# PhilippBongartz/RepeatResolver

Hardware: AMD Instinct MI355X
Metric: sum-of-pairs DP cells/sec (higher is better)
Workload: dtype u32

## Files before the change

repeatresolver_amd/csrc/pwr_device.hip:

```cpp
#include <hip/hip_runtime.h>

#include <algorithm>
#include <chrono>
#include <cstdint>
#include <cstdio>
#include <cstdlib>
#include <cstring>
#include <new>
#include <thread>
#include <type_traits>
#include <vector>

#include "pwr.h"

#define PWR_INF 0x40000000u
#define PWR_BIG 0x7fffffff

struct Hdr {
    int W;
    int nslots;
    int nfree;
    int cur;
    int status;
    int stop;
// ... 62 lines not shown
    Tally *tally;
    int *order0, *order1;
    int *rank;
    int *freelist;
    const long long *brkoff;
    const int *brkx;
    int *nbrk;
    int *hard;
    int *inscnt;
    int *newidx;
    int *bplan;
};
#define PLAN_MAX 16
#define JR_BASE (1 + 2 * PLAN_MAX)
#define BPLAN_WORDS (JR_BASE + 64 * 4)
#define PLAN_CAND 128
#define PLAN_EVRATE_MAX 12.0f
#define PLAN_SLACK 2048

#define SEG_MAX 256
struct SegDesc {
    int job, s;
    int xb, xown, xe;
    int fin, active;
    int grow0;
    unsigned long long cells;
};
struct GatherPart;
struct CommitJob {
    int nchg, nev, ndel, first;
    int u0, u1;
    int scanned, pad;
};
struct BatchPlan;
struct CommitEv;
struct JobBufs {
    GatherPart *gpart;
    unsigned gather_tag;
    JobMeta *meta;
    int *way;
    int4 *rec2;
    uint8_t *mark;
    uint8_t *mark2;
    uint32_t *dirs;
    int *newcol;
    int *aux;
    uint4 *desc;
    int wpNW, wpMS;
    unsigned *lastM;
    unsigned long long *gmb;
    SegDesc *seg;
    unsigned *chk;
    int seg_align;
    int src_start;
    int smax, seg_rows, warm_cols;
    int seg_budget, seg_minrows;
    int seg_balance;
    int plan_ahead;
    int hard_rows, hard_up, hard_down;
    int plan_len;
    int plan_gate_rel;
    int spec_inorder;
    int fail_stops;
    int plan_slack, plan_evrate_x100;
    const int *rowids;
    int gstride;
    unsigned tagbase;
    unsigned long long *gtr;
    int trk;
    unsigned trace_tag;
    long long *g64;
    int force64;
    int evcap;
    int gate_v2;
    int *chkdone;
    int check_in_trace, trace_ny;
    int trace_prior;
    int trace_blk;
    int v2_follows, f64_follows;
    int stall_test;
    unsigned long long *diag;
    int njobs_launched;
    int Lmax, colcap, NC;
    size_t dirstride;
    int split_rank, split_world;
    CommitJob *cjob;
    int *chg;
    int *evkey, *evdl;
    int *insidx;
    int *pair_cf, *pair_left;
    BatchPlan *plan;
    CommitEv *sev;
    int *freed;
    unsigned *ticket;
};
#define NOT_MINE(JB, JOB) ((JB).split_world > 1 && (JOB) % (JB).split_world != (JB).split_rank)

#define DPP_ROW_SHR(n) (0x110 + (n))
#define DPP_ROW_BCAST15 0x142
#define DPP_ROW_BCAST31 0x143
#define DPP_WAVE_SHR1 0x138

__device__ __forceinline__ int wave_incl_min(int v)
{
    int t;
    t = __builtin_amdgcn_update_dpp(PWR_BIG, v, DPP_ROW_SHR(1), 0xF, 0xF, false); v = min(v, t);
    t = __builtin_amdgcn_update_dpp(PWR_BIG, v, DPP_ROW_SHR(2), 0xF, 0xF, false); v = min(v, t);
    t = __builtin_amdgcn_update_dpp(PWR_BIG, v, DPP_ROW_SHR(4), 0xF, 0xF, false); v = min(v, t);
    t = __builtin_amdgcn_update_dpp(PWR_BIG, v, DPP_ROW_SHR(8), 0xF, 0xF, false); v = min(v, t);
    t = __builtin_amdgcn_update_dpp(PWR_BIG, v, DPP_ROW_BCAST15, 0xA, 0xF, false); v = min(v, t);
    t = __builtin_amdgcn_update_dpp(PWR_BIG, v, DPP_ROW_BCAST31, 0xC, 0xF, false); v = min(v, t);
    return v;
}
__device__ __forceinline__ int row_incl_min(int v)
{
    int t;
    t = __builtin_amdgcn_update_dpp(PWR_BIG, v, DPP_ROW_SHR(1), 0xF, 0xF, false); v = min(v, t);
    t = __builtin_amdgcn_update_dpp(PWR_BIG, v, DPP_ROW_SHR(2), 0xF, 0xF, false); v = min(v, t);
    t = __builtin_amdgcn_update_dpp(PWR_BIG, v, DPP_ROW_SHR(4), 0xF, 0xF, false); v = min(v, t);
    t = __builtin_amdgcn_update_dpp(PWR_BIG, v, DPP_ROW_SHR(8), 0xF, 0xF, false); v = min(v, t);
    return v;
}
__device__ __forceinline__ unsigned wave_incl_add(unsigned v)
{
    unsigned t;
    t = __builtin_amdgcn_update_dpp(0u, v, DPP_ROW_SHR(1), 0xF, 0xF, false); v += t;
// ... 2524 lines not shown
        for (int j = lane; j < nch; j += 64)
            tot += (int)((__hip_atomic_load(&hand[j], __ATOMIC_RELAXED, __HIP_MEMORY_SCOPE_AGENT) >> 41) & 0x7full);
        for (int o = 32; o > 0; o >>= 1) tot += __shfl_xor(tot, o);
        if (lane == 0) m->nnew = tot;
    }
#undef TB_POST
}

#define COMMIT_NT 1024
#define EVCAP 1024
#define MAXJ 128
#define CS_G 16
#define CA_G 32

__device__ __forceinline__ int row_symbol(const uint8_t *mk, int y, int lo, int y0, int y1)
{
    if (y < y0 || y > y1) return 5;
    const int v = mk[y - lo];
    return v == 7 ? 5 : (v ? v - 1 : 4);
}

enum { V_NONE = 0, V_COMMIT, V_STALE, V_STOP_NOTOK, V_STOP_GROW, V_STOP_WIDE, V_STOP_ABORT, V_STOP_SEGFAIL, V_EMPTY, V_AFTER_STOP };
struct BatchPlan {
    int idle;
    int ncommit, nnew, ndel, nev;
    int restructure, big;
    int live_all, live_done, ahead_n;
    int first;
    unsigned long long done_mask;
    int reasons[4];
    int cjobs[MAXJ], slotbase[MAXJ];
    signed char verdict[MAXJ];
};
struct CommitEv { int key[EVCAP], dl[EVCAP], skey[EVCAP], scum[EVCAP], seg_lo[EVCAP + 1], seg_sh[EVCAP + 1], seg_pre[EVCAP + 2]; int ns, cum, nev, pad; };

__global__ __launch_bounds__(COMMIT_NT) void k_commit_scan(DState st, JobBufs jb, int njobs)
{
    __shared__ unsigned sh[COMMIT_NT / 64];
    constexpr int CPQ = (PWR_MAX_SEQ_LENGTH / TB_C + COMMIT_NT) / COMMIT_NT;
    __shared__ int s_cpre[COMMIT_NT * CPQ];
    __shared__ int s_ov[MAXJ], s_ovlo[MAXJ], s_ovhi[MAXJ], s_nov;
    const int job = blockIdx.x, g = blockIdx.y, tid = threadIdx.x;
    const JobMeta *m = &jb.meta[job];
    if (st.hdr->status != 0 || st.hdr->need_grow) return;
    if (!m->active || m->L <= 0 || !m->ok || m->abort || m->segfail || (m->wide && !jb.f64_follows)) return;
    const int k = m->k, L = m->L;
    if (!m->changed && st.nbrk[k] == 0) return;
    const int nch = (L + TB_C - 1) / TB_C;
    const bool chunked = jb.trace_blk != 0 && nch <= COMMIT_NT * CPQ;
    const int G = (chunked && L >= 64 * CS_G) ? CS_G : 1;
    if (g >= G) return;
    CommitJob *cj = &jb.cjob[job];
    const long long off = st.rowoff[k];
    const int lo = m->lo;
    const int *order = cur_order(st);
    const int *way = jb.way + (size_t)job * jb.Lmax;
    const int *newcol = jb.newcol + (size_t)job * jb.Lmax;
    int *aux = jb.aux + (size_t)job * jb.Lmax;
    int *insidx = jb.insidx + (size_t)job * jb.Lmax;
    const uint8_t *mark = jb.mark + (size_t)job * jb.colcap;
    uint8_t *mark2 = jb.mark2 + (size_t)job * jb.colcap;
    int *list = jb.chg + (size_t)job * jb.colcap;
    int *evkey = jb.evkey + (size_t)job * EVCAP, *evdl = jb.evdl + (size_t)job * EVCAP;
    const int way0 = way[0], wayL = way[L - 1];
    const int nc0 = newcol[0], ncL = newcol[L - 1];
    const int ny0 = (nc0 >> 1) + (nc0 & 1), nyL = ncL >> 1;
    const int u0 = min(way0, ny0), u1 = max(wayL, nyL);
// ... 89 lines not shown
                        const int so = (y < way0 || y > wayL) ? 5 : (vo == 7 ? 5 : (vo ? vo - 1 : 4));
                        const int sn = (y < ny0 || y > nyL) ? 5 : (vn == 7 ? 5 : (vn ? vn - 1 : 4));
                        const bool chg = y >= Y0 && y < Y1 && y >= u0 && y <= u1 && so != sn;
                        ent[b] = chg ? (y | (so << 24) | (sn << 28)) : -1;
                        cnt += chg ? 1 : 0;
                    }
                }
            }
            unsigned tot;
            const unsigned incl = block_incl_add<COMMIT_NT>((unsigned)cnt, sh, tot);
            if (tid == 0 && tot) s_base = atomicAdd(&cj->nchg, (int)tot);
            __syncthreads();
            if (cnt) {
                int w_ = s_base + (int)(incl - (unsigned)cnt);
#pragma unroll
                for (int b = 0; b < 8; ++b) {
                    if (ent[b] < 0) continue;
                    const int e_ = ent[b];
                    const int y = e_ & 0xffffff, so = (e_ >> 24) & 15, sn = (e_ >> 28) & 15;
                    list[w_++] = e_;
                    touch(y, 0);
                    if (so < 4 && sn >= 4 && st.tally[order[y]].w[4] == 1u) {
                        event(2 * y, -1);
                        atomicAdd(&cj->ndel, 1);
                        touch(y, -1);
                    }
                }
            }
            __syncthreads();
        }
    }
}

__device__ void commit_decide(const DState &st, const JobBufs &jb, int njobs, BatchPlan *p, const JobMeta *metas, const CommitJob *cjobs, const int *pair_cf, const int *pair_left)
{
    const Hdr *h = st.hdr;
    p->idle = (h->status != 0 || h->need_grow) ? 1 : 0;
    p->ncommit = p->nnew = p->ndel = p->nev = p->restructure = p->big = 0;
    p->live_all = p->live_done = p->ahead_n = 0;
    p->first = 0x7fffffff;
    p->done_mask = 0ull;
    for (int i = 0; i < 4; ++i) p->reasons[i] = 0;
    for (int j = 0; j < njobs && j < MAXJ; ++j) p->verdict[j] = V_NONE;
    if (p->idle) return;
    const int W = h->W, H = st.H, B = st.B;
    int net = 0, evabs = 0, nskip = 0;
    int skipped[MAXJ];
    bool stopped = false;
    for (int j = 0; j < njobs && j < MAXJ; ++j) {
        const JobMeta *m = &metas[j];
        if (!m->active) break;
        if (m->L > 0) {
            p->live_all += 1;
            if (stopped) { p->verdict[j] = V_AFTER_STOP; continue; }
            if (!m->ok) { p->verdict[j] = V_STOP_NOTOK; stopped = true; continue; }
            if ((long long)W + p->nnew + m->L + 64 > st.colcap || (long long)h->nslots + p->nnew + m->L + 64 > st.slotcap) { p->verdict[j] = V_STOP_GROW; stopped = true; continue; }
            if (m->wide && !jb.f64_follows) { p->verdict[j] = V_STOP_WIDE; stopped = true; continue; }
            if (m->abort) { p->verdict[j] = V_STOP_ABORT; stopped = true; continue; }
            if (m->segfail) {
                p->verdict[j] = V_STOP_SEGFAIL;
                if (jb.fail_stops || nskip >= MAXJ) stopped = true; else skipped[nskip++] = j;
                continue;
            }
            bool good = true;
            int why = -1;
            int d = 0, r = 0;
            for (int t = 0; t < p->ncommit && good; ++t) {
                const int i = p->cjobs[t];
                const CommitJob *ci = &cjobs[i];
                if (!ci->scanned) continue;
                if (pair_cf[(size_t)i * njobs + j]) { good = false; why = 3; break; }
                const int neti = metas[i].nnew - ci->ndel;
                int left;
                if (ci->u1 < m->lo - 1) left = neti;
                else if (m->hi + 1 < ci->u0 - 1) left = 0;
                else left = pair_left[(size_t)i * njobs + j];
                d += left; r += neti - left;
            }
            if (good && (d != 0 || r != 0)) {
                const int *way = jb.way + (size_t)j * jb.Lmax;
// ... 5 lines not shown
            }
            for (int t = 0; t < nskip && good; ++t) {
                const JobMeta *ms = &metas[skipped[t]];
                if (!(m->hi + 2 + evabs < ms->lo || ms->hi + 2 + evabs < m->lo)) good = false;
            }
            const bool jumped = st.bplan[0] && j < PLAN_MAX && st.bplan[1 + PLAN_MAX + j] != 0x7fffffff;
            if (good && jumped && st.bplan[1 + PLAN_MAX + j] <= 2 + evabs) good = false;
            if (!good) {
                if (why >= 0) p->reasons[why] += 1;
                if (nskip >= MAXJ) { p->verdict[j] = V_AFTER_STOP; stopped = true; continue; }
                skipped[nskip++] = j;
                p->verdict[j] = V_STALE;
                continue;
            }
            p->verdict[j] = V_COMMIT;
            p->cjobs[p->ncommit] = j; p->slotbase[p->ncommit] = p->nnew;
            p->ncommit += 1;
            const CommitJob *cj = &cjobs[j];
            if (cj->scanned) {
                p->nnew += m->nnew; p->ndel += cj->ndel; p->nev += cj->nev;
                net += m->nnew - cj->ndel; evabs += cj->nev;
                if (m->nnew > 0 || cj->ndel > 0) { p->restructure = 1; p->first = min(p->first, cj->first); }
                if (cj->nev > EVCAP) p->big = 1;
            }
            p->live_done += 1;
            if (nskip > 0 || jumped) p->ahead_n += 1;
        } else p->verdict[j] = V_EMPTY;
        if (m->off < 64) p->done_mask |= 1ull << m->off; else stopped = true;
    }
    if (p->nev > jb.evcap || p->nev > EVCAP) p->big = 1;
    if (!p->restructure) p->big = 0;
}

__device__ void commit_sort_events(const JobBufs &jb, const BatchPlan *p, int W, CommitEv *ev)
{
    const int tid = threadIdx.x;
    int base = 0;
    for (int t = 0; t < p->ncommit; ++t) {
        const int j = p->cjobs[t];
        const CommitJob *cj = &jb.cjob[j];
        if (!cj->scanned) continue;
        const int n = min(cj->nev, EVCAP);
        for (int e = tid; e < n && base + e < EVCAP; e += COMMIT_NT) { ev->key[base + e] = jb.evkey[(size_t)j * EVCAP + e]; ev->dl[base + e] = jb.evdl[(size_t)j * EVCAP + e]; }
        base += n;
    }
    const int nev = min(base, EVCAP);
    __syncthreads();
    for (int e = tid; e < nev; e += COMMIT_NT) {
        const int ke = ev->key[e];
        int r = 0;
        for (int f = 0; f < nev; ++f) { const int kf = ev->key[f]; r += (kf < ke || (kf == ke && f < e)) ? 1 : 0; }
        ev->skey[r] = ke; ev->scum[r] = ev->dl[e];
    }
    __syncthreads();
    if (tid == 0) {
        int cum = 0, ns = 0, pre = 0;
        for (int e = 0; e < nev; ++e) {
            cum += ev->scum[e];
            ev->scum[e] = cum;
            const int lo_y = (ev->skey[e] >> 1) + 1;
            const int hi_y = e + 1 < nev ? ((ev->skey[e + 1] & 1) ? (ev->skey[e + 1] >> 1) + 1 : (ev->skey[e + 1] >> 1)) : W;
            if (cum != 0 && hi_y > lo_y) { ev->seg_lo[ns] = lo_y; ev->seg_sh[ns] = cum; ev->seg_pre[ns] = pre; pre += hi_y - lo_y; ++ns; }
        }
        ev->seg_pre[ns] = pre;
        ev->ns = ns; ev->cum = cum; ev->nev = nev;
    }
    __syncthreads();
}

__global__ __launch_bounds__(COMMIT_NT) void k_commit_apply(DState st, JobBufs jb, int njobs)
{
    __shared__ BatchPlan sp;
    __shared__ CommitEv ev;
    __shared__ JobMeta s_meta[MAXJ];
    __shared__ CommitJob s_cj[MAXJ];
    __shared__ int s_pcf[16 * 16], s_pl[16 * 16];
    const int tid = threadIdx.x;
    {
        const int nj = min(njobs, MAXJ);
        for (int i = tid; i < nj * (int)(sizeof(JobMeta) / 4); i += COMMIT_NT) reinterpret_cast<int *>(s_meta)[i] = reinterpret_cast<const int *>(jb.meta)[i];
        for (int i = tid; i < nj * (int)(sizeof(CommitJob) / 4); i += COMMIT_NT) reinterpret_cast<int *>(s_cj)[i] = reinterpret_cast<const int *>(jb.cjob)[i];
        if (njobs <= 16) for (int i = tid; i < njobs * njobs; i += COMMIT_NT) { s_pcf[i] = jb.pair_cf[i]; s_pl[i] = jb.pair_left[i]; }
        __syncthreads();
        if (tid == 0) commit_decide(st, jb, njobs, &sp, s_meta, s_cj, njobs <= 16 ? s_pcf : jb.pair_cf, njobs <= 16 ? s_pl : jb.pair_left);
    }
    __syncthreads();
    if (blockIdx.x == 0)
        for (int i = tid; i < (int)(sizeof(BatchPlan) / 4); i += COMMIT_NT) reinterpret_cast<int *>(jb.plan)[i] = reinterpret_cast<const int *>(&sp)[i];
    if (sp.idle || sp.ncommit == 0) return;
    const Hdr *h = st.hdr;
    const int W = h->W;
    const int *order = cur_order(st);
    const int nfree = h->nfree, nslots = h->nslots;
    const int take = min(sp.nnew, nfree);
    const int gt = (int)blockIdx.x * COMMIT_NT + tid, GT = (int)gridDim.x * COMMIT_NT;
    for (int t = 0; t < sp.ncommit; ++t) {
        const int job = sp.cjobs[t];
        const JobMeta *m = &jb.meta[job];
        const CommitJob *cj = &jb.cjob[job];
        if (!cj->scanned) continue;
        const int k = m->k, L = m->L;
        const long long off = st.rowoff[k];
        const int *way = jb.way + (size_t)job * jb.Lmax;
        const int *newcol = jb.newcol + (size_t)job * jb.Lmax;
        int *aux = jb.aux + (size_t)job * jb.Lmax;
        const int *insidx = jb.insidx + (size_t)job * jb.Lmax;
        for (int x = gt; x < L; x += GT) {
            const int c = newcol[x];
            const int y = c >> 1;
            int slot = order[y];
            if (c & 1) {
                const int idx = sp.slotbase[t] + insidx[x];
                slot = (idx < take) ? st.freelist[nfree - 1 - idx] : nslots + (idx - take);
                const int bs = (int)st.seq[off + x];
                const uint32_t al = (uint32_t)aux[x];
                Tally nt;
#pragma unroll
                for (int b = 0; b < 6; ++b) nt.w[b] = ((b != bs) ? 1u : 0u) + ((b != 4) ? al : 0u);
                nt.endcnt = (x == L - 1) ? 1u : 0u; nt.pad = 0;
                st.tally[slot] = nt;
                atomicAdd(&st.inscnt[y], 1);
            }
            aux[x] = slot;
            st.pos[off + x] = slot;
            if (x == L - 1) {
                const int oend = order[way[L - 1]];
                if (oend != slot) { atomicSub(&st.tally[oend].endcnt, 1u); if (!(c & 1)) atomicAdd(&st.tally[slot].endcnt, 1u); }
            }
        }
        const int nchg = cj->nchg;
        const int *list = jb.chg + (size_t)job * jb.colcap;
        for (int i = gt; i < nchg; i += GT) {
            const int e_ = list[i];
            const int y = e_ & 0xffffff, so = (e_ >> 24) & 15, sn = (e_ >> 28) & 15;
            Tally *tp = &st.tally[order[y]];
            const uint4 a = *reinterpret_cast<const uint4 *>(&tp->w[0]);
            const uint2 b2 = *reinterpret_cast<const uint2 *>(&tp->w[4]);
            uint32_t w[6] = {a.x, a.y, a.z, a.w, b2.x, b2.y};
#pragma unroll
            for (int b = 0; b < 6; ++b) w[b] = w[b] - ((so != 5 && b != so) ? 1u : 0u) + ((sn != 5 && b != sn) ? 1u : 0u);
            *reinterpret_cast<uint4 *>(&tp->w[0]) = make_uint4(w[0], w[1], w[2], w[3]);
            *reinterpret_cast<uint2 *>(&tp->w[4]) = make_uint2(w[4], w[5]);
        }
        const int nb = st.nbrk[k];
        const int *bx = st.brkx + st.brkoff[k];
        for (int i = gt; i < nb; i += GT) atomicSub(&st.tally[order[way[bx[i]]]].endcnt, 1u);
    }
    if (!sp.restructure || sp.big) return;
    commit_sort_events(jb, &sp, W, &ev);
    if (blockIdx.x == 0) {
        for (int i = tid; i < (int)(sizeof(CommitEv) / 4); i += COMMIT_NT) reinterpret_cast<int *>(jb.sev)[i] = reinterpret_cast<const int *>(&ev)[i];
        if (tid == 0) {
            int pfree = 0;
            for (int e = 0; e < ev.nev; ++e) if (!(ev.skey[e] & 1)) jb.freed[pfree++] = order[ev.skey[e] >> 1];
        }
    }
    const int ns = ev.ns, total = ev.seg_pre[ns];
    int *tmp = st.newidx;
    auto seg_of = [&](int i) { int a = 0, b = ns - 1; while (a < b) { const int mid = (a + b + 1) >> 1; if (ev.seg_pre[mid] <= i) a = mid; else b = mid - 1; } return a; };
    for (int i = gt; i < total; i += GT) { const int sgi = seg_of(i); tmp[i] = order[ev.seg_lo[sgi] + (i - ev.seg_pre[sgi])]; }
}

__global__ __launch_bounds__(COMMIT_NT) void k_commit_finish(DState st, JobBufs jb, int njobs, const int *rowids, Hdr *host_copy, unsigned host_seq)
{
    __shared__ unsigned sh[COMMIT_NT / 64];
    __shared__ int s_skey[EVCAP], s_scum[EVCAP], s_seg_lo[EVCAP + 1], s_seg_sh[EVCAP + 1], s_seg_pre[EVCAP + 2];
    __shared__ int s_last, s_free, s_w;
    __shared__ int s_pl[8], s_plo[64], s_phi[64], s_pL[64], s_pgap[64];
    __shared__ unsigned long long s_ahead, s_okm, s_jm;
    __shared__ unsigned s_ev;
    __shared__ int s_bp[JR_BASE], s_sel[PLAN_MAX + 1], s_gp[PLAN_MAX + 1];
    __shared__ __attribute__((aligned(16))) int s_hw[(sizeof(Hdr) + 3) / 4];
    __shared__ int s_cw0[PLAN_CAND], s_cwL[PLAN_CAND], s_cL[PLAN_CAND], s_oldnext, s_rowend;
    const int tid = threadIdx.x;
    Hdr *h = st.hdr;
    const BatchPlan *p = jb.plan;
    if (tid == 0) s_pl[0] = 0;
    const int W = h->W, cur = h->cur;
    const int *order = cur ? st.order1 : st.order0;
    int *norder = cur ? st.order0 : st.order1;
    const int nfree = h->nfree, nslots = h->nslots;
    const int take = min(p->nnew, nfree);
    const int gt = (int)blockIdx.x * COMMIT_NT + tid, GT = (int)gridDim.x * COMMIT_NT;
    int Wnew = W;
    if (!p->idle && p->restructure && !p->big) {
        const CommitEv *ev = jb.sev;
        const int nev = ev->nev, ns = ev->ns;
        for (int i = tid; i < nev; i += COMMIT_NT) { s_skey[i] = ev->skey[i]; s_scum[i] = ev->scum[i]; }
        for (int i = tid; i <= ns; i += COMMIT_NT) { s_seg_lo[i] = ev->seg_lo[i]; s_seg_sh[i] = ev->seg_sh[i]; s_seg_pre[i] = ev->seg_pre[i]; }
        __syncthreads();
        const int total = s_seg_pre[ns];
        const int *tmp = st.newidx;
        int *ordw = const_cast<int *>(order);
        auto seg_of = [&](int i) { int a = 0, b = ns - 1; while (a < b) { const int mid = (a + b + 1) >> 1; if (s_seg_pre[mid] <= i) a = mid; else b = mid - 1; } return a; };
        for (int i = gt; i < total; i += GT) {
            const int sgi = seg_of(i);
            const int yn = s_seg_lo[sgi] + (i - s_seg_pre[sgi]) + s_seg_sh[sgi];
            const int slot = tmp[i];
            ordw[yn] = slot; st.rank[slot] = yn;
        }
        for (int t = 0; t < p->ncommit; ++t) {
            const int job = p->cjobs[t];
            if (!jb.cjob[job].scanned || jb.meta[job].nnew == 0) continue;
            const int L = jb.meta[job].L;
            const int *newcol = jb.newcol + (size_t)job * jb.Lmax;
            const int *aux = jb.aux + (size_t)job * jb.Lmax;
            for (int x = gt; x < L; x += GT) {
                const int c = newcol[x];
                if (c & 1) {
                    const int y = c >> 1;
                    int tt = 0;
                    for (int xx = x - 1; xx >= 0 && newcol[xx] == c; --xx) ++tt;
                    int a = 0, b = nev;
                    while (a < b) { const int mid = (a + b) >> 1; if (s_skey[mid] < 2 * y) a = mid + 1; else b = mid; }
                    const int shy = a ? s_scum[a - 1] : 0;
                    const int kept = (a < nev && s_skey[a] == 2 * y) ? 0 : 1;
                    const int pnew = y + shy + kept + tt;
                    ordw[pnew] = aux[x]; st.rank[aux[x]] = pnew;
                    st.inscnt[y] = 0;
                }
            }
        }
        if (blockIdx.x == 0) for (int i = tid; i < p->ndel; i += COMMIT_NT) st.freelist[nfree - take + i] = jb.freed[i];
        Wnew = W + ev->cum;
    } else if (!p->idle && p->restructure && blockIdx.x == 0) {
        if (tid == 0) s_free = 0;
        __syncthreads();
        const int s0 = max(0, min(p->first, h->agree));
        unsigned carry = (unsigned)s0;
        for (int base = s0; base < W; base += COMMIT_NT) {
            const int y = base + tid;
            const bool valid = y < W;
            const int slot = valid ? order[y] : 0;
            const bool keep = valid && st.tally[slot].w[4] != 0;
            const unsigned ic = valid ? (unsigned)st.inscnt[y] : 0u;
            const unsigned cnt = (keep ? 1u : 0u) + ic;
            unsigned tot;
            const unsigned incl = block_incl_add<COMMIT_NT>(cnt, sh, tot);
            const int idx = (int)(carry + incl - cnt);
            carry += tot;
            if (valid) {
                st.newidx[y] = idx;
                if (keep) { norder[idx] = slot; st.rank[slot] = idx; }
                else { const int q = atomicAdd(&s_free, 1); st.freelist[nfree - take + q] = slot; }
                if (ic) st.inscnt[y] = 0;
            }
        }
        __syncthreads();
        for (int t = 0; t < p->ncommit; ++t) {
            const int job = p->cjobs[t];
            if (!jb.cjob[job].scanned || jb.meta[job].nnew == 0) continue;
            const int L = jb.meta[job].L;
            const int *newcol = jb.newcol + (size_t)job * jb.Lmax;
            const int *aux = jb.aux + (size_t)job * jb.Lmax;
            for (int x = tid; x < L; x += COMMIT_NT) {
                const int c = newcol[x];
                if (c & 1) {
                    const int y = c >> 1;
                    int tt = 0;
                    for (int xx = x - 1; xx >= 0 && newcol[xx] == c; --xx) ++tt;
                    const int keepy = st.tally[order[y]].w[4] != 0 ? 1 : 0;
                    const int q = st.newidx[y] + keepy + tt;
                    norder[q] = aux[x];
                    st.rank[aux[x]] = q;
                }
            }
        }
        if (tid == 0) s_w = (int)carry;
        __syncthreads();
        Wnew = s_w;
        if (tid == 0) jb.sev->cum = Wnew - W;
    }
    asm volatile("s_waitcnt vmcnt(0)" ::: "memory");
    __syncthreads();
    if (tid == 0) {
        __builtin_amdgcn_fence(__ATOMIC_RELEASE, "agent");
        asm volatile("s_waitcnt vmcnt(0)" ::: "memory");
        s_last = __hip_atomic_fetch_add(jb.ticket, 1u, __ATOMIC_RELAXED, __HIP_MEMORY_SCOPE_AGENT) == gridDim.x - 1 ? 1 : 0;
        if (s_last) { __builtin_amdgcn_fence(__ATOMIC_ACQUIRE, "agent"); asm volatile("s_waitcnt vmcnt(0)" ::: "memory"); }
    }
    __syncthreads();
    if (!s_last) return;
    constexpr int HW = (int)(sizeof(Hdr) / 4);
    static_assert(HW <= COMMIT_NT, "one word of the header per thread");
    if (tid < HW) s_hw[tid] = reinterpret_cast<const int *>(h)[tid];
    if (tid < JR_BASE) s_bp[tid] = st.bplan[tid];
    __syncthreads();
    Hdr *const hh = reinterpret_cast<Hdr *>(s_hw);
    if (tid == 0) { s_oldnext = hh->next_row; s_rowend = hh->row_end; }
    __syncthreads();
    if (tid >= 64 && tid < 64 + PLAN_CAND) {
        const int c_ = tid - 64, kk = s_oldnext + c_;
        int w0 = 0, wL = 0, L_ = -1;
        if (kk < s_rowend) {
            const int kr = rowids[kk];
            L_ = st.rowlen[kr];
            if (L_ > 0) { const long long offr = st.rowoff[kr]; w0 = st.rank[st.pos[offr]]; wL = st.rank[st.pos[offr + L_ - 1]]; }
        }
        s_cw0[c_] = w0; s_cwL[c_] = wL; s_cL[c_] = L_;
    }
    if (tid == 0) {
        *jb.ticket = 0u;
        hh->ncommitted = 0; hh->stop = 0;
        if (!p->idle) {
            int version = hh->version, nfail = 0;
            for (int j = 0; j < njobs && j < MAXJ; ++j) {
                const int v = p->verdict[j];
                if (v == V_NONE) break;
                JobMeta *m = &jb.meta[j];
                if (v == V_STOP_GROW) hh->need_grow = 1;
                else if (v == V_STOP_ABORT) {
                    hh->stalls += 1;
                    if (jb.wpNW <= 16) hh->fallback = 65; else atomicCAS(&hh->status, 0, PWR_ERR_STALL);
                } else if (v == V_STOP_SEGFAIL) {
                    hh->seg_fails += 1;
                    if (jb.hard_rows && m->level == 0) {
                        if (m->hard & 1) { hh->hard_fills += (m->hard & 2) ? 0 : 1; hh->hard_refail += (m->hard & 2) ? 0 : 1; }
                        else hh->hard_marked += 1;
                        st.hard[m->k] = min(1 << 20, st.hard[m->k] + jb.hard_up);
                    }
                    if (!nfail++) {
                        hh->noseg_level = hh->noseg_row == m->k ? hh->noseg_level + 1 : 1; hh->noseg_row = m->k;
                        if (hh->noseg_level == 1 && hh->warm_step > 0) hh->warm_cur = min(hh->warm_hi, hh->warm_cur + hh->warm_up);
                    } else if (hh->warm_step > 0) hh->warm_cur = min(hh->warm_hi, hh->warm_cur + hh->warm_up);
                } else if (v == V_STALE) hh->stop = 1;
                else if (v == V_COMMIT) {
                    const CommitJob *cj = &jb.cjob[j];
                    if (cj->scanned) {
                        version += 1;
                        if (cj->nchg > 0 || m->nnew > 0) hh->rows_changed += 1;
                        if (st.nbrk[m->k]) st.nbrk[m->k] = 0;
                    }
                    hh->cells_reference += m->cells;
                    if (hh->noseg_row == m->k) { hh->noseg_row = -1; hh->noseg_level = 0; }
                    else if (m->nseg > 1 && !(m->hard & 2)) hh->warm_cur = max(hh->warm_lo, hh->warm_cur - hh->warm_step);
                    if (jb.hard_rows && (m->hard & 1) && m->level == 0 && m->nseg > 1) {
                        if (!(m->hard & 2)) hh->hard_fills += 1;
                        st.hard[m->k] = max(0, st.hard[m->k] - jb.hard_down);
                    }
                    if (m->wide) hh->rows_wide += 1;
                }
            }
            hh->version = version;
            for (int i = 0; i < 4; ++i) hh->fail_reason[i] += (unsigned long long)p->reasons[i];
            if (p->restructure) {
                const int cum = jb.sev->cum;
                hh->W = W + cum;
                hh->nslots = nslots + (p->nnew - take);
                hh->nfree = nfree - take + p->ndel;
                if (!p->big) hh->agree = max(0, min(hh->agree, min(p->first, W)));
                else { hh->cur = cur ^ 1; hh->agree = max(0, min(p->first, W)); }
            }
            unsigned long long jm = hh->jumpmask;
            if (s_bp[0]) {
                for (int j = 0; j < njobs && j < PLAN_MAX; ++j) {
                    if (p->verdict[j] != V_COMMIT || s_bp[1 + PLAN_MAX + j] == 0x7fffffff) continue;
                    const JobMeta *m = &jb.meta[j];
                    if (m->off >= 64) continue;
                    const int *nc = jb.newcol + (size_t)j * jb.Lmax;
                    const int c0 = nc[0], cL = nc[m->L - 1];
                    int *rec = st.bplan + JR_BASE + 4 * ((hh->next_row + m->off) & 63);
                    rec[0] = (int)(unsigned)(hh->events_total + (unsigned long long)p->nev);
                    rec[1] = ((c0 >> 1) + (c0 & 1)) - m->lo + m->nnew + 4;
                    rec[2] = m->hi - (cL >> 1) + m->nnew + 4;
                    jm |= 1ull << m->off;
                    hh->rows_jumped += 1;
                }
            }
            hh->events_total += (unsigned long long)p->nev;
            {
                int nchg = 0;
                for (int t = 0; t < p->ncommit; ++t) nchg += jb.cjob[p->cjobs[t]].scanned ? 1 : 0;
                if (nchg > 0) hh->evrate = 0.9f * hh->evrate + 0.1f * ((float)p->nev / (float)nchg);
            }
            const unsigned long long dm = hh->ahead | p->done_mask;
            const int adv = ~dm ? __builtin_ctzll(~dm) : 64;
            hh->jumpmask = adv >= 64 ? 0ull : jm >> adv;
            const int done = __builtin_popcountll(p->done_mask);
            hh->ncommitted = done;
            hh->next_row += adv;
            hh->ahead = adv >= 64 ? 0ull : dm >> adv;
            hh->rows_ahead += (unsigned long long)p->ahead_n;
            if (hh->fallback > 0 && jb.v2_follows) hh->fallback -= 1;
            if (hh->need64 > 0 && jb.f64_follows) hh->need64 -= 1;
            if (p->live_all > 0) hh->batches += 1;
            hh->rows_committed += (unsigned long long)p->live_done;
            hh->rows_recomputed += (unsigned long long)(p->live_all - p->live_done);
            if (hh->status == 0 && !hh->need_grow && done > 0) {
                const float ema = 0.75f * hh->ema + 0.25f * (float)done;
                hh->ema = ema;
                const int k = hh->next_row, left = hh->row_end - k;
                int nb = (int)(ema + 2.6f);
                nb = max(1, min(nb, min(hh->window, left)));
                if (left > 0) {
                    const int l0 = st.rowlen[rowids[k]];
                    for (int j = 1; j < nb; ++j)
                        if (st.rowlen[rowids[k + j]] > l0 + (int)((long long)l0 * hh->speclen / 100) + 64) { nb = j; break; }
                }
                hh->nb = nb;
                s_pl[0] = (jb.plan_ahead && hh->window > 1 && hh->window <= PLAN_MAX && left > 0) ? 1 : 0;
                s_pl[1] = k; s_pl[2] = hh->row_end; s_pl[3] = nb; s_pl[4] = min(hh->window, left); s_pl[5] = hh->W; s_pl[6] = hh->speclen;
                s_ahead = hh->ahead;
                s_pl[7] = hh->evrate * 100.0f < fminf((float)jb.plan_evrate_x100, jb.plan_gate_rel ? (float)jb.plan_slack * (100.0f / 128.0f) : 3.0e38f) ? 1 : 0;
                s_jm = hh->jumpmask; s_ev = (unsigned)hh->events_total;
                if (!s_pl[0]) st.bplan[0] = 0;
// ... 518 lines not shown
    if ((rc = dmalloc(c, &jb.lastM, (size_t)njobs * jb.NC))) return rc;
    jb.smax = std::max(1, std::min(c->seg_max, SEG_MAX));
    jb.hard_up = std::max(1, (int)((long long)c->B * c->hard_up_pm / 1000)); jb.hard_down = (int)((long long)c->B * c->hard_down_pm / 1000);
    jb.rowids = c->d_rowids;
    jb.seg_rows = c->fill_mode == 4 ? c->seg_rows : 0;
    jb.split_rank = c->split_rank; jb.split_world = c->split_world;
    jb.warm_cols = (int)std::min<long long>((long long)c->B * c->warm_pct / 100 + 2, 1 << 20);
    jb.gstride = jb.Lmax + jb.smax * (2 * jb.warm_cols + 64);
    if ((rc = dmalloc(c, &jb.seg, (size_t)njobs * SEG_MAX))) return rc;
    if (hipMemsetAsync(jb.seg, 0, sizeof(SegDesc) * (size_t)njobs * SEG_MAX, c->stream) != hipSuccess) return PWR_ERR_DEVICE;
    if ((rc = dmalloc(c, &jb.chk, (size_t)njobs * (SEG_MAX + 1) * 2 * NC))) return rc;
    if (hipMemsetAsync(jb.chk, 0xff, sizeof(unsigned) * (size_t)njobs * (SEG_MAX + 1) * 2 * NC, c->stream) != hipSuccess) return PWR_ERR_DEVICE;
    if (c->fill_mode == 4) {
        const size_t nmb = (size_t)njobs * NW * jb.gstride;
        if ((rc = dmalloc(c, &jb.gmb, nmb))) return rc;
        if (hipMemsetAsync(jb.gmb, 0, nmb * 8, c->stream) != hipSuccess ||
            hipStreamSynchronize(c->stream) != hipSuccess) return PWR_ERR_DEVICE;
        c->fill_epoch = 0;
    }
    jb.trk = std::max(TRK, jb.Lmax / TB_C + 1);
    if ((rc = dmalloc(c, &jb.gtr, (size_t)njobs * jb.trk))) return rc;
    if ((rc = dmalloc(c, &jb.diag, (size_t)njobs * 32 * 4096))) return rc;
    if (hipMemsetAsync(jb.diag, 0, (size_t)njobs * 32 * 4096 * 8, c->stream) != hipSuccess) return PWR_ERR_DEVICE;
    if (hipMemsetAsync(jb.gtr, 0, (size_t)njobs * jb.trk * 8, c->stream) != hipSuccess) return PWR_ERR_DEVICE;
    c->trace_epoch = 0;
    if ((rc = dmalloc(c, &c->d_jobrows, njobs))) return rc;
    if ((rc = dmalloc(c, &jb.cjob, njobs))) return rc;
    if ((rc = dmalloc(c, &jb.chg, (size_t)njobs * jb.colcap))) return rc;
    if ((rc = dmalloc(c, &jb.evkey, (size_t)njobs * EVCAP))) return rc;
    if ((rc = dmalloc(c, &jb.evdl, (size_t)njobs * EVCAP))) return rc;
    if ((rc = dmalloc(c, &jb.insidx, (size_t)njobs * jb.Lmax))) return rc;
    if ((rc = dmalloc(c, &jb.pair_cf, (size_t)njobs * njobs))) return rc;
    if ((rc = dmalloc(c, &jb.pair_left, (size_t)njobs * njobs))) return rc;
    if ((rc = dmalloc(c, &jb.plan, 1))) return rc;
    if ((rc = dmalloc(c, &jb.sev, 1))) return rc;
    if ((rc = dmalloc(c, &jb.freed, EVCAP))) return rc;
    if ((rc = dmalloc(c, &jb.ticket, 4))) return rc;
    if ((rc = dmalloc(c, &jb.chkdone, (size_t)njobs))) return rc;
    if (hipMemsetAsync(jb.chkdone, 0, sizeof(int) * (size_t)njobs, c->stream) != hipSuccess) return PWR_ERR_DEVICE;
    if (hipMemsetAsync(jb.cjob, 0, sizeof(CommitJob) * njobs, c->stream) != hipSuccess || hipMemsetAsync(jb.pair_cf, 0, sizeof(int) * (size_t)njobs * njobs, c->stream) != hipSuccess ||
        hipMemsetAsync(jb.pair_left, 0, sizeof(int) * (size_t)njobs * njobs, c->stream) != hipSuccess || hipMemsetAsync(jb.plan, 0, sizeof(BatchPlan), c->stream) != hipSuccess ||
        hipMemsetAsync(jb.sev, 0, sizeof(CommitEv), c->stream) != hipSuccess || hipMemsetAsync(jb.ticket, 0, 16, c->stream) != hipSuccess) return PWR_ERR_DEVICE;
    if (hipMemset(jb.meta, 0, sizeof(JobMeta) * njobs) != hipSuccess) return PWR_ERR_DEVICE;
    c->job_allocs.assign(c->allocs.begin() + first, c->allocs.end());
    c->njobs = njobs;
    return PWR_OK;
}

static void free_jobs(pwr_ctx *c)
{
    for (void *p : c->job_allocs) dfree(c, p);
    c->job_allocs.clear();
    c->jb = JobBufs{};
    c->d_jobrows = nullptr;
    c->njobs = 0;
}

static int upload(pwr_ctx *c)
{
    if (c->on_device) return PWR_OK;
    const int T = c->T, W0 = c->W_host;
    if (hipSetDevice(c->device) != hipSuccess) return PWR_ERR_DEVICE;
    std::vector<uint32_t> w((size_t)W0 * 6, 0);
    std::vector<long long> rowoff(T + 1, 0);
    c->rowlen.assign(T, 0);
    {
        const unsigned nth = par_threads(T);
        std::vector<std::vector<uint32_t>> cnt(nth, std::vector<uint32_t>((size_t)W0 * 6, 0));
        std::vector<int> errs(nth, 0);
        par_rows(T, [&](int r0, int r1, int t) {
            uint32_t *ct = cnt[t].data();
            for (int r = r0; r < r1; ++r) {
                const unsigned char *row = &c->text[(size_t)r * W0];
                int L = 0;
                for (int i = 0; i < W0; ++i) {
// ... 297 lines not shown
    return h.status;
}

static int enqueue_front(pwr_ctx *c)
{
    const int n = c->window;
    int rc;
    c->jb.gather_tag = ++c->gather_tag;
    c->jb.rowids = c->d_rowids;
    c->jb.f64_follows = (c->seen_need64 > 0 || c->force64) ? 1 : 0;
    hipLaunchKernelGGL(k_gather_a, dim3(n, GATHER_G), dim3(GATHER_NT), 0, c->stream, c->st, c->jb, c->d_rowids);
    hipLaunchKernelGGL(k_gather_c, dim3(n, GATHER_G + 1), dim3(GATHER_NT), 0, c->stream, c->st, c->jb);
    c->jb.trace_ny = (c->jb.Lmax / TB_C + TB_W) / TB_W;
    c->jb.check_in_trace = (c->check_in_trace && c->fill_mode == 4 && c->par_trace == 2 && c->st.colcap < TB_MAXCOL && c->jb.smax > 1 && c->jb.seg_rows > 0) ? 1 : 0;
    if ((rc = launch_fill(c, n))) return rc;
    if (c->jb.f64_follows) hipLaunchKernelGGL(k_fill64, dim3(n), dim3(F64_NT), 0, c->stream, c->st, c->jb);
    if (c->par_trace) {
        if (++c->trace_epoch >= (1 << 14)) { HIPC(hipMemsetAsync(c->jb.gtr, 0, (size_t)c->njobs * c->jb.trk * 8, c->stream)); c->trace_epoch = 1; }
        c->jb.trace_tag = (unsigned)c->trace_epoch;
        c->jb.trace_blk = (c->par_trace == 2 && c->st.colcap < TB_MAXCOL) ? 1 : 0;
        c->jb.trace_prior = c->trace_prior;
        if (c->jb.trace_blk) hipLaunchKernelGGL(k_trace_blk, dim3(n, c->jb.trace_ny + (c->jb.check_in_trace ? c->jb.smax - 1 : 0)), dim3(TB_W * 64), 0, c->stream, c->st, c->jb);
        else hipLaunchKernelGGL(k_trace_par, dim3(n, TRK / TRW), dim3(TRW * 64), 0, c->stream, c->st, c->jb);
    }
    else { c->jb.trace_blk = 0; hipLaunchKernelGGL(k_trace_wp, dim3(n), dim3(64), 0, c->stream, c->st, c->jb); }
    HIPC(hipGetLastError());
    return PWR_OK;
}

static int enqueue_commit(pwr_ctx *c, Hdr *host_copy, unsigned host_seq)
{
    const int n = c->window;
    hipLaunchKernelGGL(k_commit_scan, dim3(n, CS_G), dim3(COMMIT_NT), 0, c->stream, c->st, c->jb, n);
    hipLaunchKernelGGL(k_commit_apply, dim3(CA_G), dim3(COMMIT_NT), 0, c->stream, c->st, c->jb, n);
    hipLaunchKernelGGL(k_commit_finish, dim3(CA_G), dim3(COMMIT_NT), 0, c->stream, c->st, c->jb, n, c->d_rowids, host_copy, host_seq);
    HIPC(hipGetLastError());
    return PWR_OK;
}

static int enqueue_batch(pwr_ctx *c, Hdr *host_copy, unsigned host_seq)
{
    int rc = enqueue_front(c);
    if (rc) return rc;
    return enqueue_commit(c, host_copy, host_seq);
}

#define PWR_INFLIGHT 3
#define PWR_POLL_LIMIT_S 120

static int slab_init(pwr_ctx *c, int k0, int n)
{
    const int kend = k0 + n;
    int nb = (int)(c->batch_ema + 2.6);
    nb = std::max(1, std::min(nb, std::min(c->window, n)));
    for (int j = 1; j < nb; ++j)
        if (c->rowlen[c->ids[k0 + j]] > c->rowlen[c->ids[k0]] + (int)((long long)c->rowlen[c->ids[k0]] * c->spec_len / 100) + 64) { nb = j; break; }
    const float ema0 = (float)c->batch_ema;
    struct { int next_row, row_end, nb, need_grow, window; } init = {k0, kend, nb, 0, c->window};
    static_assert(sizeof(init) == offsetof(Hdr, fallback) - offsetof(Hdr, next_row), "slab fields of Hdr");
    HIPC(hipMemcpyAsync(&c->st.hdr->ema, &ema0, sizeof(float), hipMemcpyHostToDevice, c->stream));
    HIPC(hipMemcpyAsync(&c->st.hdr->speclen, &c->spec_len, sizeof(int), hipMemcpyHostToDevice, c->stream));
    HIPC(hipMemcpyAsync(&c->st.hdr->next_row, &init, sizeof init, hipMemcpyHostToDevice, c->stream));
    HIPC(hipMemsetAsync(&c->st.hdr->ahead, 0, sizeof(unsigned long long), c->stream));
    HIPC(hipMemsetAsync(c->st.bplan, 0, sizeof(int), c->stream));
    HIPC(hipMemsetAsync(&c->st.hdr->jumpmask, 0, sizeof(unsigned long long), c->stream));
    HIPC(hipStreamSynchronize(c->stream));
    return PWR_OK;
// ... 475 lines not shown
```

Baseline: 58.62 billion.

## Fuse commit apply into finish kernel with double-buffered order remap

Merges k_commit_apply into k_commit_finish so each block recomputes the batch plan and event sort in shared memory, removing one kernel launch and the global plan/event/freed staging buffers. The fast restructure path now writes a full remapped order into the alternate order buffer (norder) via per-row binary search over events, instead of a segment gather to a temporary followed by an in-place scatter. The header always flips cur on restructure. In exchange every block redundantly runs commit_decide and the event sort, and the fast path touches all rows from s0 to W rather than only the shifted segments.

```diff
diff --git a/repeatresolver_amd/csrc/pwr_device.hip b/repeatresolver_amd/csrc/pwr_device.hip
--- a/repeatresolver_amd/csrc/pwr_device.hip
+++ b/repeatresolver_amd/csrc/pwr_device.hip
@@ -118,8 +118,6 @@
     int u0, u1;
     int scanned, pad;
 };
-struct BatchPlan;
-struct CommitEv;
 struct JobBufs {
     GatherPart *gpart;
     unsigned gather_tag;
@@ -175,9 +173,6 @@
     int *evkey, *evdl;
     int *insidx;
     int *pair_cf, *pair_left;
-    BatchPlan *plan;
-    CommitEv *sev;
-    int *freed;
     unsigned *ticket;
 };
 #define NOT_MINE(JB, JOB) ((JB).split_world > 1 && (JOB) % (JB).split_world != (JB).split_rank)
@@ -2768,7 +2763,7 @@
     int cjobs[MAXJ], slotbase[MAXJ];
     signed char verdict[MAXJ];
 };
-struct CommitEv { int key[EVCAP], dl[EVCAP], skey[EVCAP], scum[EVCAP], seg_lo[EVCAP + 1], seg_sh[EVCAP + 1], seg_pre[EVCAP + 2]; int ns, cum, nev, pad; };
+struct CommitEv { int key[EVCAP], dl[EVCAP], skey[EVCAP], scum[EVCAP], del[EVCAP]; int cum, nev, ndel, pad; };
 
 __global__ __launch_bounds__(COMMIT_NT) void k_commit_scan(DState st, JobBufs jb, int njobs)
 {
@@ -2924,7 +2919,7 @@
     }
 }
 
-__device__ void commit_decide(const DState &st, const JobBufs &jb, int njobs, BatchPlan *p, const JobMeta *metas, const CommitJob *cjobs, const int *pair_cf, const int *pair_left)
+__device__ void commit_decide(const DState &st, const JobBufs &jb, int njobs, BatchPlan *p, const JobMeta *metas, const CommitJob *cjobs, const int *pair_cf, const int *pair_left, int *skipped)
 {
     const Hdr *h = st.hdr;
     p->idle = (h->status != 0 || h->need_grow) ? 1 : 0;
@@ -2937,7 +2932,6 @@
     if (p->idle) return;
     const int W = h->W, H = st.H, B = st.B;
     int net = 0, evabs = 0, nskip = 0;
-    int skipped[MAXJ];
     bool stopped = false;
     for (int j = 0; j < njobs && j < MAXJ; ++j) {
         const JobMeta *m = &metas[j];
@@ -3009,13 +3003,13 @@
     if (!p->restructure) p->big = 0;
 }
 
-__device__ void commit_sort_events(const JobBufs &jb, const BatchPlan *p, int W, CommitEv *ev)
+__device__ void commit_sort_events(const JobBufs &jb, const BatchPlan *p, const CommitJob *cjobs, CommitEv *ev)
 {
     const int tid = threadIdx.x;
     int base = 0;
     for (int t = 0; t < p->ncommit; ++t) {
         const int j = p->cjobs[t];
-        const CommitJob *cj = &jb.cjob[j];
+        const CommitJob *cj = &cjobs[j];
         if (!cj->scanned) continue;
         const int n = min(cj->nev, EVCAP);
         for (int e = tid; e < n && base + e < EVCAP; e += COMMIT_NT) { ev->key[base + e] = jb.evkey[(size_t)j * EVCAP + e]; ev->dl[base + e] = jb.evdl[(size_t)j * EVCAP + e]; }
@@ -3031,50 +3025,62 @@
     }
     __syncthreads();
     if (tid == 0) {
-        int cum = 0, ns = 0, pre = 0;
+        int cum = 0, ndel = 0;
         for (int e = 0; e < nev; ++e) {
             cum += ev->scum[e];
             ev->scum[e] = cum;
-            const int lo_y = (ev->skey[e] >> 1) + 1;
-            const int hi_y = e + 1 < nev ? ((ev->skey[e + 1] & 1) ? (ev->skey[e + 1] >> 1) + 1 : (ev->skey[e + 1] >> 1)) : W;
-            if (cum != 0 && hi_y > lo_y) { ev->seg_lo[ns] = lo_y; ev->seg_sh[ns] = cum; ev->seg_pre[ns] = pre; pre += hi_y - lo_y; ++ns; }
-        }
-        ev->seg_pre[ns] = pre;
-        ev->ns = ns; ev->cum = cum; ev->nev = nev;
+            if (!(ev->skey[e] & 1)) ev->del[ndel++] = ev->skey[e] >> 1;
+        }
+        ev->cum = cum; ev->nev = nev; ev->ndel = ndel;
     }
     __syncthreads();
 }
 
-__global__ __launch_bounds__(COMMIT_NT) void k_commit_apply(DState st, JobBufs jb, int njobs)
+__global__ __launch_bounds__(COMMIT_NT) void k_commit_finish(DState st, JobBufs jb, int njobs, const int *rowids, Hdr *host_copy, unsigned host_seq)
 {
     __shared__ BatchPlan sp;
     __shared__ CommitEv ev;
     __shared__ JobMeta s_meta[MAXJ];
     __shared__ CommitJob s_cj[MAXJ];
-    __shared__ int s_pcf[16 * 16], s_pl[16 * 16];
+    __shared__ int s_pcf[16 * 16], s_plf[16 * 16], s_skip[MAXJ];
+    __shared__ unsigned sh[COMMIT_NT / 64];
+    __shared__ int s_last, s_free, s_w;
+    __shared__ int s_pl[8], s_plo[64], s_phi[64], s_pL[64], s_pgap[64];
+    __shared__ unsigned long long s_ahead, s_okm, s_jm;
+    __shared__ unsigned s_ev;
+    __shared__ int s_bp[JR_BASE], s_sel[PLAN_MAX + 1], s_gp[PLAN_MAX + 1];
+    __shared__ __attribute__((aligned(16))) int s_hw[(sizeof(Hdr) + 3) / 4];
+    __shared__ int s_cw0[PLAN_CAND], s_cwL[PLAN_CAND], s_cL[PLAN_CAND], s_oldnext, s_rowend;
     const int tid = threadIdx.x;
+    Hdr *h = st.hdr;
+    const BatchPlan *p = &sp;
+    if (tid == 0) s_pl[0] = 0;
+    const int W = h->W, cur = h->cur, agree = h->agree;
+    const int nfree = h->nfree, nslots = h->nslots;
+    const int *order = cur ? st.order1 : st.order0;
+    int *norder = cur ? st.order0 : st.order1;
     {
         const int nj = min(njobs, MAXJ);
         for (int i = tid; i < nj * (int)(sizeof(JobMeta) / 4); i += COMMIT_NT) reinterpret_cast<int *>(s_meta)[i] = reinterpret_cast<const int *>(jb.meta)[i];
         for (int i = tid; i < nj * (int)(sizeof(CommitJob) / 4); i += COMMIT_NT) reinterpret_cast<int *>(s_cj)[i] = reinterpret_cast<const int *>(jb.cjob)[i];
-        if (njobs <= 16) for (int i = tid; i < njobs * njobs; i += COMMIT_NT) { s_pcf[i] = jb.pair_cf[i]; s_pl[i] = jb.pair_left[i]; }
+        if (njobs <= 16) for (int i = tid; i < njobs * njobs; i += COMMIT_NT) { s_pcf[i] = jb.pair_cf[i]; s_plf[i] = jb.pair_left[i]; }
         __syncthreads();
-        if (tid == 0) commit_decide(st, jb, njobs, &sp, s_meta, s_cj, njobs <= 16 ? s_pcf : jb.pair_cf, njobs <= 16 ? s_pl : jb.pair_left);
+        if (tid == 0) commit_decide(st, jb, njobs, &sp, s_meta, s_cj, njobs <= 16 ? s_pcf : jb.pair_cf, njobs <= 16 ? s_plf : jb.pair_left, s_skip);
     }
     __syncthreads();
-    if (blockIdx.x == 0)
-        for (int i = tid; i < (int)(sizeof(BatchPlan) / 4); i += COMMIT_NT) reinterpret_cast<int *>(jb.plan)[i] = reinterpret_cast<const int *>(&sp)[i];
-    if (sp.idle || sp.ncommit == 0) return;
-    const Hdr *h = st.hdr;
-    const int W = h->W;
-    const int *order = cur_order(st);
-    const int nfree = h->nfree, nslots = h->nslots;
     const int take = min(sp.nnew, nfree);
     const int gt = (int)blockIdx.x * COMMIT_NT + tid, GT = (int)gridDim.x * COMMIT_NT;
-    for (int t = 0; t < sp.ncommit; ++t) {
+    const bool work = !sp.idle && sp.ncommit > 0;
+    const bool fast = work && sp.restructure && !sp.big;
+    constexpr int CPY = 4;
+    const int s0 = max(0, min(sp.first, agree));
+    int cslot[CPY];
+#pragma unroll
+    for (int u = 0; u < CPY; ++u) { const int y = s0 + gt + u * GT; cslot[u] = (fast && y < W) ? order[y] : 0; }
+    for (int t = 0; work && t < sp.ncommit; ++t) {
         const int job = sp.cjobs[t];
-        const JobMeta *m = &jb.meta[job];
-        const CommitJob *cj = &jb.cjob[job];
+        const JobMeta *m = &s_meta[job];
+        const CommitJob *cj = &s_cj[job];
         if (!cj->scanned) continue;
         const int k = m->k, L = m->L;
         const long long off = st.rowoff[k];
@@ -3096,7 +3102,7 @@
                 for (int b = 0; b < 6; ++b) nt.w[b] = ((b != bs) ? 1u : 0u) + ((b != 4) ? al : 0u);
                 nt.endcnt = (x == L - 1) ? 1u : 0u; nt.pad = 0;
                 st.tally[slot] = nt;
-                atomicAdd(&st.inscnt[y], 1);
+                if (sp.big) atomicAdd(&st.inscnt[y], 1);
             }
             aux[x] = slot;
             st.pos[off + x] = slot;
@@ -3123,63 +3129,24 @@
         const int *bx = st.brkx + st.brkoff[k];
         for (int i = gt; i < nb; i += GT) atomicSub(&st.tally[order[way[bx[i]]]].endcnt, 1u);
     }
-    if (!sp.restructure || sp.big) return;
-    commit_sort_events(jb, &sp, W, &ev);
-    if (blockIdx.x == 0) {
-        for (int i = tid; i < (int)(sizeof(CommitEv) / 4); i += COMMIT_NT) reinterpret_cast<int *>(jb.sev)[i] = reinterpret_cast<const int *>(&ev)[i];
-        if (tid == 0) {
-            int pfree = 0;
-            for (int e = 0; e < ev.nev; ++e) if (!(ev.skey[e] & 1)) jb.freed[pfree++] = order[ev.skey[e] >> 1];
-        }
-    }
-    const int ns = ev.ns, total = ev.seg_pre[ns];
-    int *tmp = st.newidx;
-    auto seg_of = [&](int i) { int a = 0, b = ns - 1; while (a < b) { const int mid = (a + b + 1) >> 1; if (ev.seg_pre[mid] <= i) a = mid; else b = mid - 1; } return a; };
-    for (int i = gt; i < total; i += GT) { const int sgi = seg_of(i); tmp[i] = order[ev.seg_lo[sgi] + (i - ev.seg_pre[sgi])]; }
-}
-
-__global__ __launch_bounds__(COMMIT_NT) void k_commit_finish(DState st, JobBufs jb, int njobs, const int *rowids, Hdr *host_copy, unsigned host_seq)
-{
-    __shared__ unsigned sh[COMMIT_NT / 64];
-    __shared__ int s_skey[EVCAP], s_scum[EVCAP], s_seg_lo[EVCAP + 1], s_seg_sh[EVCAP + 1], s_seg_pre[EVCAP + 2];
-    __shared__ int s_last, s_free, s_w;
-    __shared__ int s_pl[8], s_plo[64], s_phi[64], s_pL[64], s_pgap[64];
-    __shared__ unsigned long long s_ahead, s_okm, s_jm;
-    __shared__ unsigned s_ev;
-    __shared__ int s_bp[JR_BASE], s_sel[PLAN_MAX + 1], s_gp[PLAN_MAX + 1];
-    __shared__ __attribute__((aligned(16))) int s_hw[(sizeof(Hdr) + 3) / 4];
-    __shared__ int s_cw0[PLAN_CAND], s_cwL[PLAN_CAND], s_cL[PLAN_CAND], s_oldnext, s_rowend;
-    const int tid = threadIdx.x;
-    Hdr *h = st.hdr;
-    const BatchPlan *p = jb.plan;
-    if (tid == 0) s_pl[0] = 0;
-    const int W = h->W, cur = h->cur;
-    const int *order = cur ? st.order1 : st.order0;
-    int *norder = cur ? st.order0 : st.order1;
-    const int nfree = h->nfree, nslots = h->nslots;
-    const int take = min(p->nnew, nfree);
-    const int gt = (int)blockIdx.x * COMMIT_NT + tid, GT = (int)gridDim.x * COMMIT_NT;
-    int Wnew = W;
-    if (!p->idle && p->restructure && !p->big) {
-        const CommitEv *ev = jb.sev;
-        const int nev = ev->nev, ns = ev->ns;
-        for (int i = tid; i < nev; i += COMMIT_NT) { s_skey[i] = ev->skey[i]; s_scum[i] = ev->scum[i]; }
-        for (int i = tid; i <= ns; i += COMMIT_NT) { s_seg_lo[i] = ev->seg_lo[i]; s_seg_sh[i] = ev->seg_sh[i]; s_seg_pre[i] = ev->seg_pre[i]; }
-        __syncthreads();
-        const int total = s_seg_pre[ns];
-        const int *tmp = st.newidx;
-        int *ordw = const_cast<int *>(order);
-        auto seg_of = [&](int i) { int a = 0, b = ns - 1; while (a < b) { const int mid = (a + b + 1) >> 1; if (s_seg_pre[mid] <= i) a = mid; else b = mid - 1; } return a; };
-        for (int i = gt; i < total; i += GT) {
-            const int sgi = seg_of(i);
-            const int yn = s_seg_lo[sgi] + (i - s_seg_pre[sgi]) + s_seg_sh[sgi];
-            const int slot = tmp[i];
-            ordw[yn] = slot; st.rank[slot] = yn;
-        }
+    if (fast) {
+        commit_sort_events(jb, &sp, s_cj, &ev);
+        const int nev = ev.nev;
+        auto place = [&](int y, int slot) {
+            int a = 0, b = nev;
+            while (a < b) { const int mid = (a + b) >> 1; if (ev.skey[mid] < 2 * y) a = mid + 1; else b = mid; }
+            if (a < nev && ev.skey[a] == 2 * y) return;
+            const int shy = a ? ev.scum[a - 1] : 0;
+            norder[y + shy] = slot;
+            if (shy) st.rank[slot] = y + shy;
+        };
+#pragma unroll
+        for (int u = 0; u < CPY; ++u) { const int y = s0 + gt + u * GT; if (y < W) place(y, cslot[u]); }
+        for (int y = s0 + gt + CPY * GT; y < W; y += GT) place(y, order[y]);
         for (int t = 0; t < p->ncommit; ++t) {
             const int job = p->cjobs[t];
-            if (!jb.cjob[job].scanned || jb.meta[job].nnew == 0) continue;
-            const int L = jb.meta[job].L;
+            if (!s_cj[job].scanned || s_meta[job].nnew == 0) continue;
+            const int L = s_meta[job].L;
             const int *newcol = jb.newcol + (size_t)job * jb.Lmax;
             const int *aux = jb.aux + (size_t)job * jb.Lmax;
             for (int x = gt; x < L; x += GT) {
@@ -3189,21 +3156,31 @@
                     int tt = 0;
                     for (int xx = x - 1; xx >= 0 && newcol[xx] == c; --xx) ++tt;
                     int a = 0, b = nev;
-                    while (a < b) { const int mid = (a + b) >> 1; if (s_skey[mid] < 2 * y) a = mid + 1; else b = mid; }
-                    const int shy = a ? s_scum[a - 1] : 0;
-                    const int kept = (a < nev && s_skey[a] == 2 * y) ? 0 : 1;
+                    while (a < b) { const int mid = (a + b) >> 1; if (ev.skey[mid] < 2 * y) a = mid + 1; else b = mid; }
+                    const int shy = a ? ev.scum[a - 1] : 0;
+                    const int kept = (a < nev && ev.skey[a] == 2 * y) ? 0 : 1;
                     const int pnew = y + shy + kept + tt;
-                    ordw[pnew] = aux[x]; st.rank[aux[x]] = pnew;
-                    st.inscnt[y] = 0;
+                    norder[pnew] = aux[x]; st.rank[aux[x]] = pnew;
                 }
             }
         }
-        if (blockIdx.x == 0) for (int i = tid; i < p->ndel; i += COMMIT_NT) st.freelist[nfree - take + i] = jb.freed[i];
-        Wnew = W + ev->cum;
-    } else if (!p->idle && p->restructure && blockIdx.x == 0) {
+    }
+    asm volatile("s_waitcnt vmcnt(0)" ::: "memory");
+    __syncthreads();
+    if (tid == 0) {
+        __builtin_amdgcn_fence(__ATOMIC_RELEASE, "agent");
+        asm volatile("s_waitcnt vmcnt(0)" ::: "memory");
+        s_last = __hip_atomic_fetch_add(jb.ticket, 1u, __ATOMIC_RELAXED, __HIP_MEMORY_SCOPE_AGENT) == gridDim.x - 1 ? 1 : 0;
+        if (s_last) { __builtin_amdgcn_fence(__ATOMIC_ACQUIRE, "agent"); asm volatile("s_waitcnt vmcnt(0)" ::: "memory"); }
+    }
+    __syncthreads();
+    if (!s_last) return;
+    if (fast) {
+        for (int i = tid; i < ev.ndel; i += COMMIT_NT) st.freelist[nfree - take + i] = order[ev.del[i]];
+        if (tid == 0) s_w = W + ev.cum;
+    } else if (work && sp.restructure) {
         if (tid == 0) s_free = 0;
         __syncthreads();
-        const int s0 = max(0, min(p->first, h->agree));
         unsigned carry = (unsigned)s0;
         for (int base = s0; base < W; base += COMMIT_NT) {
             const int y = base + tid;
@@ -3226,8 +3203,8 @@
         __syncthreads();
         for (int t = 0; t < p->ncommit; ++t) {
             const int job = p->cjobs[t];
-            if (!jb.cjob[job].scanned || jb.meta[job].nnew == 0) continue;
-            const int L = jb.meta[job].L;
+            if (!s_cj[job].scanned || s_meta[job].nnew == 0) continue;
+            const int L = s_meta[job].L;
             const int *newcol = jb.newcol + (size_t)job * jb.Lmax;
             const int *aux = jb.aux + (size_t)job * jb.Lmax;
             for (int x = tid; x < L; x += COMMIT_NT) {
@@ -3244,20 +3221,7 @@
             }
         }
         if (tid == 0) s_w = (int)carry;
-        __syncthreads();
-        Wnew = s_w;
-        if (tid == 0) jb.sev->cum = Wnew - W;
-    }
-    asm volatile("s_waitcnt vmcnt(0)" ::: "memory");
-    __syncthreads();
-    if (tid == 0) {
-        __builtin_amdgcn_fence(__ATOMIC_RELEASE, "agent");
-        asm volatile("s_waitcnt vmcnt(0)" ::: "memory");
-        s_last = __hip_atomic_fetch_add(jb.ticket, 1u, __ATOMIC_RELAXED, __HIP_MEMORY_SCOPE_AGENT) == gridDim.x - 1 ? 1 : 0;
-        if (s_last) { __builtin_amdgcn_fence(__ATOMIC_ACQUIRE, "agent"); asm volatile("s_waitcnt vmcnt(0)" ::: "memory"); }
-    }
-    __syncthreads();
-    if (!s_last) return;
+    }
     constexpr int HW = (int)(sizeof(Hdr) / 4);
     static_assert(HW <= COMMIT_NT, "one word of the header per thread");
     if (tid < HW) s_hw[tid] = reinterpret_cast<const int *>(h)[tid];
@@ -3284,7 +3248,7 @@
             for (int j = 0; j < njobs && j < MAXJ; ++j) {
                 const int v = p->verdict[j];
                 if (v == V_NONE) break;
-                JobMeta *m = &jb.meta[j];
+                const JobMeta *m = &s_meta[j];
                 if (v == V_STOP_GROW) hh->need_grow = 1;
                 else if (v == V_STOP_ABORT) {
                     hh->stalls += 1;
@@ -3302,7 +3266,7 @@
                     } else if (hh->warm_step > 0) hh->warm_cur = min(hh->warm_hi, hh->warm_cur + hh->warm_up);
                 } else if (v == V_STALE) hh->stop = 1;
                 else if (v == V_COMMIT) {
-                    const CommitJob *cj = &jb.cjob[j];
+                    const CommitJob *cj = &s_cj[j];
                     if (cj->scanned) {
                         version += 1;
                         if (cj->nchg > 0 || m->nnew > 0) hh->rows_changed += 1;
@@ -3321,18 +3285,16 @@
             hh->version = version;
             for (int i = 0; i < 4; ++i) hh->fail_reason[i] += (unsigned long long)p->reasons[i];
             if (p->restructure) {
-                const int cum = jb.sev->cum;
-                hh->W = W + cum;
+                hh->W = s_w;
                 hh->nslots = nslots + (p->nnew - take);
                 hh->nfree = nfree - take + p->ndel;
-                if (!p->big) hh->agree = max(0, min(hh->agree, min(p->first, W)));
-                else { hh->cur = cur ^ 1; hh->agree = max(0, min(p->first, W)); }
+                hh->cur = cur ^ 1; hh->agree = max(0, min(p->first, W));
             }
             unsigned long long jm = hh->jumpmask;
             if (s_bp[0]) {
                 for (int j = 0; j < njobs && j < PLAN_MAX; ++j) {
                     if (p->verdict[j] != V_COMMIT || s_bp[1 + PLAN_MAX + j] == 0x7fffffff) continue;
-                    const JobMeta *m = &jb.meta[j];
+                    const JobMeta *m = &s_meta[j];
                     if (m->off >= 64) continue;
                     const int *nc = jb.newcol + (size_t)j * jb.Lmax;
                     const int c0 = nc[0], cL = nc[m->L - 1];
@@ -3347,7 +3309,7 @@
             hh->events_total += (unsigned long long)p->nev;
             {
                 int nchg = 0;
-                for (int t = 0; t < p->ncommit; ++t) nchg += jb.cjob[p->cjobs[t]].scanned ? 1 : 0;
+                for (int t = 0; t < p->ncommit; ++t) nchg += s_cj[p->cjobs[t]].scanned ? 1 : 0;
                 if (nchg > 0) hh->evrate = 0.9f * hh->evrate + 0.1f * ((float)p->nev / (float)nchg);
             }
             const unsigned long long dm = hh->ahead | p->done_mask;
@@ -3932,15 +3894,12 @@
     if ((rc = dmalloc(c, &jb.insidx, (size_t)njobs * jb.Lmax))) return rc;
     if ((rc = dmalloc(c, &jb.pair_cf, (size_t)njobs * njobs))) return rc;
     if ((rc = dmalloc(c, &jb.pair_left, (size_t)njobs * njobs))) return rc;
-    if ((rc = dmalloc(c, &jb.plan, 1))) return rc;
-    if ((rc = dmalloc(c, &jb.sev, 1))) return rc;
-    if ((rc = dmalloc(c, &jb.freed, EVCAP))) return rc;
     if ((rc = dmalloc(c, &jb.ticket, 4))) return rc;
     if ((rc = dmalloc(c, &jb.chkdone, (size_t)njobs))) return rc;
     if (hipMemsetAsync(jb.chkdone, 0, sizeof(int) * (size_t)njobs, c->stream) != hipSuccess) return PWR_ERR_DEVICE;
     if (hipMemsetAsync(jb.cjob, 0, sizeof(CommitJob) * njobs, c->stream) != hipSuccess || hipMemsetAsync(jb.pair_cf, 0, sizeof(int) * (size_t)njobs * njobs, c->stream) != hipSuccess ||
-        hipMemsetAsync(jb.pair_left, 0, sizeof(int) * (size_t)njobs * njobs, c->stream) != hipSuccess || hipMemsetAsync(jb.plan, 0, sizeof(BatchPlan), c->stream) != hipSuccess ||
-        hipMemsetAsync(jb.sev, 0, sizeof(CommitEv), c->stream) != hipSuccess || hipMemsetAsync(jb.ticket, 0, 16, c->stream) != hipSuccess) return PWR_ERR_DEVICE;
+        hipMemsetAsync(jb.pair_left, 0, sizeof(int) * (size_t)njobs * njobs, c->stream) != hipSuccess ||
+        hipMemsetAsync(jb.ticket, 0, 16, c->stream) != hipSuccess) return PWR_ERR_DEVICE;
     if (hipMemset(jb.meta, 0, sizeof(JobMeta) * njobs) != hipSuccess) return PWR_ERR_DEVICE;
     c->job_allocs.assign(c->allocs.begin() + first, c->allocs.end());
     c->njobs = njobs;
@@ -4304,7 +4263,6 @@
 {
     const int n = c->window;
     hipLaunchKernelGGL(k_commit_scan, dim3(n, CS_G), dim3(COMMIT_NT), 0, c->stream, c->st, c->jb, n);
-    hipLaunchKernelGGL(k_commit_apply, dim3(CA_G), dim3(COMMIT_NT), 0, c->stream, c->st, c->jb, n);
     hipLaunchKernelGGL(k_commit_finish, dim3(CA_G), dim3(COMMIT_NT), 0, c->stream, c->st, c->jb, n, c->d_rowids, host_copy, host_seq);
     HIPC(hipGetLastError());
     return PWR_OK;
```

Measured after the change: 60.28 billion, median of 6. 2.8% higher.
